# MiloszKrajewski/K4os.Compression.LZ4

Hardware: NVIDIA H100
Metric: GB/s uncompressed (encode+decode) on batched 64KiB blocks @1/2/4/8 GPU vs CPU ref (higher is better)
Workload: dtype u8

## Files before the change

k4os/compression/lz4_b200/csrc/encode_generic.cuh:

```cuda
#pragma once
#include "common.cuh"

namespace k4 {

constexpr int ENC_TABLE_BYTES = 16384;
constexpr int ENC_FLAG_X32 = 0x100;
#ifndef K4_ENC_TAGS
#define K4_ENC_TAGS 0
#endif
constexpr int ENC_TAG_BYTES = K4_ENC_TAGS ? 8192 : 0;
constexpr int ENC_SLOT_BYTES = ENC_TABLE_BYTES + ENC_TAG_BYTES;
#ifndef K4_ENC_GTAG
#define K4_ENC_GTAG 2
#endif
constexpr int ENC_GTAG = K4_ENC_GTAG;
constexpr int ENC_GSLOT_BYTES = ENC_GTAG == 2 ? 2 * ENC_TABLE_BYTES : (ENC_GTAG ? ENC_TABLE_BYTES + ENC_TABLE_BYTES / 2 : ENC_TABLE_BYTES);

struct EncCtx {
    const uint8_t* src;
    uint32_t n;
    bool by16;
    bool use5;
    uint16_t* t16;
    uint32_t* t32;
    __device__ __forceinline__ uint32_t hash_at(uint32_t p) const {
        if (by16) return hash4(ldg_u32u(src + p), 13);
        return use5 ? hash5(ldg_u64u(src + p), 12) : hash4(ldg_u32u(src + p), 12);
    }
    __device__ __forceinline__ uint32_t tget(uint32_t h) const { return by16 ? (uint32_t)t16[h] : t32[h]; }
    __device__ __forceinline__ void tput(uint32_t h, uint32_t v) const {
        if (by16) t16[h] = (uint16_t)v; else t32[h] = v;
    }
};

__device__ __forceinline__ uint32_t run_header_size(uint32_t run) {
    return run >= 15 ? 2 + (run - 15) / 255 : 1;
}
__device__ __forceinline__ void write_run_header(uint8_t* dst, uint32_t op, uint32_t run) {
    if (run >= 15) {
        uint32_t rest = run - 15;
        dst[op++] = 0xF0;
        for (; rest >= 255; rest -= 255) dst[op++] = 255;
        dst[op++] = (uint8_t)rest;
    } else {
        dst[op] = (uint8_t)(run << 4);
    }
}

__device__ int encode_block_warp(const uint8_t* __restrict__ src, int n_, uint8_t* __restrict__ dst,
                                 int cap, int hardCap, void* tableSmem, bool enforce32) {
    const int lane = lane_id();
    if ((uint32_t)n_ > (uint32_t)MAX_INPUT_SIZE) return 0;
    EncCtx c;
    c.src = src; c.n = (uint32_t)n_;
    c.by16 = n_ < LIMIT_64K;
    c.use5 = !c.by16 && !enforce32;
    c.t16 = reinterpret_cast<uint16_t*>(tableSmem);
    c.t32 = reinterpret_cast<uint32_t*>(tableSmem);
    const bool limited = !(cap >= max_output_size(n_));
    const int64_t olimit = cap;
    const int64_t hard = hardCap;
    const uint32_t n = c.n;

    {
        uint4* t = reinterpret_cast<uint4*>(tableSmem);
        for (int i = lane; i < ENC_TABLE_BYTES / 16; i += 32) t[i] = make_uint4(0, 0, 0, 0);
        __syncwarp();
    }

    uint32_t ip = 0, anchor = 0, op = 0;

    if (n >= (uint32_t)MINLENGTH) {
        const uint32_t mfl1 = n - MFLIMIT + 1;
        const uint32_t mlim = n - LASTLITERALS;
        uint32_t fh = 0, m = 0, tokpos = 0;
        if (lane == 0) {
            c.tput(c.hash_at(0), 0);
            fh = c.hash_at(1);
        }
        ip = 1;
        for (;;) {
            uint32_t status = 0;
            if (lane == 0) {
                uint32_t fwd = ip, step = 1, cnt = 1u << SKIP_TRIGGER;
                for (;;) {
                    const uint32_t hh = fh, cur = fwd;
                    m = c.tget(hh);
                    ip = fwd;
                    fwd += step;
                    step = cnt++ >> SKIP_TRIGGER;
                    if (fwd > mfl1) { status = 0; break; }
                    fh = c.hash_at(fwd);
                    c.tput(hh, cur);
                    if (!c.by16 && m + MAX_DISTANCE < cur) continue;
                    if (ldg_u32u(src + m) == ldg_u32u(src + ip)) { status = 1; break; }
                }
                if (status) {
                    while (ip > anchor && m > 0 && __ldg(src + ip - 1) == __ldg(src + m - 1)) { ip--; m--; }
                }
            }
            status = __shfl_sync(FULL, status, 0);
            if (!status) break;
            ip = __shfl_sync(FULL, ip, 0);
            m = __shfl_sync(FULL, m, 0);

            {
                const uint32_t lit = ip - anchor;
                if (limited && (int64_t)op + 1 + lit + 8 + lit / 255 > olimit) return 0;
                const uint32_t hdr = run_header_size(lit);
                if ((int64_t)op + hdr + lit > hard) return 0;
                tokpos = op;
                if (lane == 0) write_run_header(dst, op, lit);
                op += hdr;
                for (uint32_t i = lane; i < lit; i += 32) dst[op + i] = __ldg(src + anchor + i);
                op += lit;
            }

            for (;;) {
                if ((int64_t)op + 2 > hard) return 0;
                if (lane == 0) { dst[op] = (uint8_t)(ip - m); dst[op + 1] = (uint8_t)((ip - m) >> 8); }
                op += 2;
                uint32_t mc = 0;
                {
                    uint32_t a = ip + MINMATCH, b = m + MINMATCH;
                    for (;;) {
                        const bool in = a + lane < mlim;
                        const bool eq = in && (__ldg(src + a + lane) == __ldg(src + b + lane));
                        const unsigned miss = __ballot_sync(FULL, !eq);
                        if (miss) { mc += __ffs(miss) - 1; break; }
                        mc += 32; a += 32; b += 32;
                    }
                }
                ip += mc + MINMATCH;
                if (limited && (int64_t)op + 6 + (mc + 240) / 255 > olimit) return 0;
                if (mc >= 15) {
                    const uint32_t rest = mc - 15;
                    const uint32_t nff = rest / 255;
                    if ((int64_t)op + nff + 1 > hard) return 0;
                    for (uint32_t i = lane; i < nff; i += 32) dst[op + i] = 0xFF;
                    if (lane == 0) {
                        dst[tokpos] = (uint8_t)(dst[tokpos] + 15);
                        dst[op + nff] = (uint8_t)(rest % 255);
                    }
                    op += nff + 1;
                } else if (lane == 0) {
                    dst[tokpos] = (uint8_t)(dst[tokpos] + mc);
                }
                __syncwarp();
                anchor = ip;
                if (ip >= mfl1) goto last_literals;

                uint32_t hit = 0;
                if (lane == 0) {
                    c.tput(c.hash_at(ip - 2), ip - 2);
                    const uint32_t hh = c.hash_at(ip);
                    m = c.tget(hh);
                    c.tput(hh, ip);
                    if ((c.by16 || m + MAX_DISTANCE >= ip) && ldg_u32u(src + m) == ldg_u32u(src + ip))
                        hit = 1;
                    else
                        fh = c.hash_at(ip + 1);
                }
                hit = __shfl_sync(FULL, hit, 0);
                if (!hit) { ip++; break; }
                m = __shfl_sync(FULL, m, 0);
                if ((int64_t)op + 1 > hard) return 0;
                tokpos = op;
                if (lane == 0) dst[op] = 0;
                op++;
                __syncwarp();
            }
        }
    }

last_literals:
    {
        const uint32_t run = n - anchor;
        if (limited && (int64_t)op + run + 1 + (run + 255 - 15) / 255 > olimit) return 0;
        const uint32_t hdr = run_header_size(run);
        if ((int64_t)op + hdr + run > hard) return 0;
        if (lane == 0) write_run_header(dst, op, run);
        op += hdr;
        for (uint32_t i = lane; i < run; i += 32) dst[op + i] = __ldg(src + anchor + i);
        op += run;
    }
    return (int)op;
}

__device__ __forceinline__ int codec_encode_warp(const uint8_t* src, int n, uint8_t* dst, int cap,
                                                 int level, void* table, bool enforce32) {
    if (n <= 0) return 0;
    if (level >= 3) return -2;
    int r = encode_block_warp(src, n, dst, cap, 0x7fffffff, table, enforce32);
    return r <= 0 ? -1 : r;
}

constexpr int ENC_WARPS_PER_CTA = K4_ENC_TAGS ? 9 : 7;
#ifndef K4_ENC_SM_WARPS
#define K4_ENC_SM_WARPS 8
#endif
#ifndef K4_ENC_GM_WARPS
#define K4_ENC_GM_WARPS 22
#endif
constexpr int ENC_SM_WARPS = K4_ENC_SM_WARPS;
constexpr int ENC_GM_WARPS = K4_ENC_GM_WARPS;

}
```

k4os/compression/lz4_b200/csrc/encode_tile.cuh:

```cuda
#pragma once
#include "common.cuh"
#include "encode_generic.cuh"

namespace k4 {


__device__ __forceinline__ uint32_t lds_u32u(const uint8_t* p) {
    const uintptr_t a = reinterpret_cast<uintptr_t>(p);
    const uint32_t* w = reinterpret_cast<const uint32_t*>(a & ~uintptr_t(3));
    return __funnelshift_r(w[0], w[1], (uint32_t)(a & 3) * 8);
}

#ifndef K4_ENC_OVL
#define K4_ENC_OVL 1
#endif
#ifndef K4_ENC_PF
#define K4_ENC_PF 0
#endif
__device__ __forceinline__ void prefetch_l1(const void* p) { asm volatile("prefetch.global.L1 [%0];" :: "l"(p)); }

__device__ __forceinline__ uint32_t probe_advance(uint32_t q) {
    if (q <= 64u) return q;
    if (q == 0) return 0;
    const uint32_t c = 63u + q, k = c >> 6;
    return 1u + 32u * k * (k - 1u) + (c - 64u * k) * k;
}

template <bool STAGED, bool HARD = true, bool GTAB = false, int TAGMODE = (K4_ENC_TAGS ? 1 : 0)>
__device__ int encode_spec_warp(const uint8_t* __restrict__ src, const uint8_t* sin, const uint32_t n,
                                uint8_t* __restrict__ dst, const int cap, const int hardCap, uint16_t* table) {
    const int lane = lane_id();
    const int64_t hard = hardCap;
#define RD32(p) (STAGED ? lds_u32u(sin + (p)) : ldg_u32u(src + (p)))
#ifndef K4_ENC_GTAB_L1
#define K4_ENC_GTAB_L1 0
#endif
#define TGET(h) ((GTAB && !K4_ENC_GTAB_L1) ? (uint32_t)__ldcg(table + (h)) : (uint32_t)table[(h)])
    constexpr bool TAGS = TAGMODE != 0;
    constexpr uint32_t TAG_SHIFT = TAGMODE == 2 ? 3u : 11u, TAG_MASK = TAGMODE == 2 ? 0xFFFFu : 0xFFu;
    uint8_t* const tags = reinterpret_cast<uint8_t*>(table) + ENC_TABLE_BYTES;
    uint32_t* const table32 = reinterpret_cast<uint32_t*>(table);
    auto tagGet = [&](uint32_t h) -> uint32_t {
        return (GTAB && !K4_ENC_GTAB_L1) ? (uint32_t)__ldcg(tags + h) : (uint32_t)tags[h];
    };
    auto slotPut = [&](uint32_t h, uint32_t pos, uint32_t tg) {
        if (TAGMODE == 2) {
            if (GTAB) __stcg(table32 + h, pos | (tg << 16)); else table32[h] = pos | (tg << 16);
        } else {
            if (GTAB && !K4_ENC_GTAB_L1) __stcg(table + h, (uint16_t)pos); else table[h] = (uint16_t)pos;
            if (TAGS) { if (GTAB && !K4_ENC_GTAB_L1) __stcg(tags + h, (uint8_t)tg); else tags[h] = (uint8_t)tg; }
        }
    };
#define RD8(p) (STAGED ? (uint32_t)sin[(p)] : (uint32_t)__ldg(src + (p)))
    {
        const uint32_t t0 = (TAGS && n >= 4) ? (((RD32(0) * 2654435761u) >> TAG_SHIFT) & TAG_MASK) : 0u;
        const uint32_t fillT = TAGMODE == 2 ? (t0 << 16) : 0u;
        uint4* t = reinterpret_cast<uint4*>(table);
        constexpr int TBYTES = TAGMODE == 2 ? 2 * ENC_TABLE_BYTES : ENC_TABLE_BYTES;
        for (int i = lane; i < TBYTES / 16; i += 32) {
            if (GTAB) __stcg(t + i, make_uint4(fillT, fillT, fillT, fillT)); else t[i] = make_uint4(fillT, fillT, fillT, fillT);
        }
        if (TAGMODE == 1 || TAGMODE == 3) {
            const uint32_t b4 = t0 * 0x01010101u;
            uint4* g = reinterpret_cast<uint4*>(tags);
            for (int i = lane; i < (ENC_TABLE_BYTES / 2) / 16; i += 32) {
                if (GTAB) __stcg(g + i, make_uint4(b4, b4, b4, b4)); else g[i] = make_uint4(b4, b4, b4, b4);
            }
        }
        __syncwarp();
    }
    const bool limited = !(cap >= max_output_size((int)n));
    const int64_t olimit = cap;
    uint32_t ip = 0, anchor = 0, op = 0;

    if (n >= (uint32_t)MINLENGTH) {
        const uint32_t mfl1 = n - MFLIMIT + 1, mlim = n - LASTLITERALS;
        if (lane == 0) { const uint32_t p0 = RD32(0) * 2654435761u; slotPut(p0 >> 19, 0u, (p0 >> TAG_SHIFT) & TAG_MASK); }
        __syncwarp();
        ip = 1;
        bool post = false;
        uint32_t q0 = 0;
        uint32_t base = 1;
        for (;;) {
            uint32_t h2 = 0xFFFFFFFFu, tag2 = 0;
            if (post) { const uint32_t p2 = RD32(ip - 2) * 2654435761u; h2 = p2 >> 19; tag2 = (p2 >> TAG_SHIFT) & TAG_MASK; }
            const bool isPost = post && lane == 0;
            const uint32_t q = q0 + (uint32_t)lane - (post ? 1u : 0u);
            const uint32_t pos = isPost ? ip : base + probe_advance(q);
            const bool valid = isPost || (base + probe_advance(q + 1) <= mfl1);
            const uint32_t v = valid ? RD32(pos) : 0u;
            const uint32_t prod = v * 2654435761u;
            const uint32_t h = valid ? prod >> 19 : (0x10000u + (uint32_t)lane);
            const uint32_t tg = (prod >> TAG_SHIFT) & TAG_MASK;
            uint32_t cand = 0u, ctag = tg;
            bool lazyPos = false;
            if (TAGMODE == 2) {
                const uint32_t e32 = valid ? ((GTAB && !K4_ENC_GTAB_L1) ? __ldcg(table32 + h) : table32[h]) : 0xFFFF0000u;
                cand = e32 & 0xFFFFu; ctag = e32 >> 16;
                if (!valid) ctag = 0x10000u;
            } else if (TAGMODE == 3) {
                ctag = valid ? tagGet(h) : 0x100u;
                lazyPos = true;
            } else {
                cand = valid ? TGET(h) : 0u;
                if (TAGMODE == 1) ctag = valid ? tagGet(h) : 0x100u;
            }
            if (h == h2) { cand = ip - 2; ctag = TAGS ? tag2 : tg; lazyPos = false; }
            const unsigned peers = __match_any_sync(FULL, h);
            const unsigned earlier = peers & ((1u << lane) - 1u);
            const int fromLane = earlier ? 31 - __clz(earlier) : lane;
            const uint32_t fwdPos = __shfl_sync(FULL, pos, fromLane);
            const uint32_t fwdTag = __shfl_sync(FULL, tg, fromLane);
            if (earlier) { cand = fwdPos; ctag = TAGS ? fwdTag : tg; lazyPos = false; }
            bool hit = false;
            if (valid && ctag == tg) {
                if (TAGMODE == 3 && lazyPos) cand = TGET(h);
                hit = RD32(cand) == v;
                if (TAGS && !STAGED && (K4_ENC_PF & 1)) {
                    prefetch_l1(src + (cand + 32u < n ? cand + 32u : n - 1u));
                    if (cand >= 8u) prefetch_l1(src + cand - 8u);
                }
            }
            if (!STAGED && (K4_ENC_PF & 2) && lane == 0) prefetch_l1(src + (pos + 384u < n ? pos + 384u : n - 1u));
            const unsigned hits = __ballot_sync(FULL, hit);
            const unsigned ends = __ballot_sync(FULL, !valid);
            const int f = hits ? __ffs(hits) - 1 : 32;
            const int e = ends ? __ffs(ends) - 1 : 32;
            if (e < f) break;
            {
                const unsigned upto = (f >= 31) ? 0xffffffffu : ((2u << f) - 1u);
                const unsigned later = peers & ~((2u << lane) - 1u) & upto;
                const bool doStore = valid && ((1u << lane) & upto) && !(lane < 31 ? later : 0u);
                if (post) {
                    const unsigned same2 = __ballot_sync(FULL, valid && h == h2) & upto;
                    if (lane == 0 && !same2) {
                        slotPut(h2, ip - 2, tag2);
                    }
                }
                if (doStore) slotPut(h, pos, tg);
                __syncwarp();
            }
            if (f == 32) {
                if (post) { post = false; base = ip + 1; q0 = 31; }
                else q0 += 32;
                continue;
            }
            const bool zeroLit = post && f == 0;
            uint32_t m = __shfl_sync(FULL, cand, f);
            ip = __shfl_sync(FULL, pos, f);
            const uint32_t a0h = ip + MINMATCH, b0h = m + MINMATCH;
            uint32_t x1 = 0u;
            if (K4_ENC_OVL) {
                const uint32_t a = a0h + 4u * lane;
                if (lane < 8 && (int)mlim - (int)a > 0) x1 = RD32(a) ^ RD32(b0h + 4u * lane);
            }
            uint32_t caught = 0;
            if (!zeroLit) {
                for (int width = 8;; width = 32) {
                    const bool part = lane < width;
                    const bool ok = !part || ((ip > anchor + lane) && (m > (uint32_t)lane) &&
                                              (RD8(ip - 1 - lane) == RD8(m - 1 - lane)));
                    const unsigned bad = __ballot_sync(FULL, !ok);
                    const int c = bad ? __ffs(bad) - 1 : width;
                    ip -= c; m -= c; caught += (uint32_t)c;
                    if (bad) break;
                }
            }
            const uint32_t lit = ip - anchor;
            if (!zeroLit && limited && (int64_t)op + 1 + lit + 8 + lit / 255 > olimit) return 0;
            uint32_t mc = caught;
            {
                uint32_t a0 = a0h, b0 = b0h;
                for (int width = 8;; width = 32) {
                    const uint32_t a = a0 + 4u * lane, bb = b0 + 4u * lane;
                    const bool part = lane < width;
                    const int room = (int)mlim - (int)a;
                    const uint32_t x = (K4_ENC_OVL && width == 8) ? x1 : ((part && room > 0) ? (RD32(a) ^ RD32(bb)) : 0u);
                    int eq = x ? ((__ffs(x) - 1) >> 3) : 4;
                    if (eq > room) eq = room < 0 ? 0 : room;
                    if (!part) eq = 4;
                    const unsigned stop = __ballot_sync(FULL, eq < 4);
                    if (stop) {
                        const int s = __ffs(stop) - 1;
                        mc += 4u * s + (uint32_t)__shfl_sync(FULL, eq, s);
                        break;
                    }
                    mc += 4u * width; a0 += 4u * width; b0 += 4u * width;
                }
            }
            const uint32_t hdr = run_header_size(lit);
            const uint32_t afterOff = op + hdr + lit + 2;
            if (limited && (int64_t)afterOff + 6 + (mc + 240) / 255 > olimit) return 0;
            if (HARD && (int64_t)afterOff + (mc >= 15 ? (mc - 15) / 255 + 1 : 0) > hard) return 0;
            {
                const uint32_t mlTok = mc >= 15 ? 15u : mc;
                if (lane == 0) {
                    if (lit >= 15) {
                        uint32_t o = op, rest = lit - 15;
                        dst[o++] = (uint8_t)(0xF0 | mlTok);
                        for (; rest >= 255; rest -= 255) dst[o++] = 255;
                        dst[o] = (uint8_t)rest;
                    } else dst[op] = (uint8_t)((lit << 4) | mlTok);
                    dst[afterOff - 2] = (uint8_t)(ip - m);
                    dst[afterOff - 1] = (uint8_t)((ip - m) >> 8);
                }
                for (uint32_t i = lane; i < lit; i += 32) dst[op + hdr + i] = RD8(anchor + i);
                op = afterOff;
                if (mc >= 15) {
                    const uint32_t rest = mc - 15, nff = rest / 255;
                    for (uint32_t i = lane; i < nff; i += 32) dst[op + i] = 0xFF;
                    if (lane == 0) dst[op + nff] = (uint8_t)(rest % 255);
                    op += nff + 1;
                }
            }
            ip += mc + MINMATCH;
            anchor = ip;
            if (ip >= mfl1) break;
            post = true; q0 = 0; base = ip + 1;
        }
    }
    {
        const uint32_t run = n - anchor;
        if (limited && (int64_t)op + run + 1 + (run + 255 - 15) / 255 > olimit) return 0;
        const uint32_t hdr = run_header_size(run);
        if (HARD && (int64_t)op + hdr + run > hard) return 0;
        if (lane == 0) write_run_header(dst, op, run);
        op += hdr;
        for (uint32_t i = lane; i < run; i += 32) dst[op + i] = RD8(anchor + i);
        op += run;
        return (int)op;
    }
#undef RD32
#undef TGET
#undef RD8
}

__device__ unsigned long long g_encode_stats[4];

template <bool GTAB>
__device__ __forceinline__ void encode_persistent_warp(
        const uint8_t* __restrict__ srcBase, const int64_t* __restrict__ srcOff,
        const int32_t* __restrict__ srcLen, uint8_t* __restrict__ dstBase,
        const int64_t* __restrict__ dstOff, const int32_t* __restrict__ dstCap,
        int32_t* __restrict__ outLen, const int nBlocks, int level,
        uint32_t* __restrict__ nextBlock, uint16_t* const table, const int reserve) {
    const int lane = lane_id();
    const bool enforce32 = (level & ENC_FLAG_X32) != 0;
    level &= 0xFF;
    for (;;) {
        int b = 0;
        if (lane == 0) {
            if (GTAB && (int)*(volatile uint32_t*)nextBlock >= nBlocks - reserve) b = nBlocks;
            else b = (int)atomicAdd(nextBlock, 1u);
        }
        b = __shfl_sync(FULL, b, 0);
        if (b >= nBlocks) return;
        const int n_ = srcLen[b];
        const uint8_t* __restrict__ src = srcBase + srcOff[b];
        uint8_t* __restrict__ dst = dstBase + dstOff[b];
        const int cap = dstCap[b];
        if (n_ <= 0) { if (lane == 0) outLen[b] = 0; continue; }
        if (level >= 3) { if (lane == 0) outLen[b] = -2; continue; }
        int r;
        if (n_ >= LIMIT_64K) r = encode_block_warp(src, n_, dst, cap, 0x7fffffff, table, enforce32);
        else r = encode_spec_warp<false, false, GTAB, GTAB ? ENC_GTAG : (K4_ENC_TAGS ? 1 : 0)>(src, nullptr, (uint32_t)n_, dst, cap, 0x7fffffff, table);
        if (lane == 0) {
            outLen[b] = r <= 0 ? -1 : r;
            atomicAdd(&g_encode_stats[n_ >= LIMIT_64K ? 2 : (GTAB ? 1 : 0)], 1ull);
        }
        __syncwarp();
    }
}

__global__ void __launch_bounds__(32)
encode_spec_kernel(const uint8_t* __restrict__ srcBase, const int64_t* __restrict__ srcOff,
                   const int32_t* __restrict__ srcLen, uint8_t* __restrict__ dstBase,
                   const int64_t* __restrict__ dstOff, const int32_t* __restrict__ dstCap,
                   int32_t* __restrict__ outLen, int nBlocks, int level, uint32_t* __restrict__ nextBlock) {
    extern __shared__ __align__(128) uint8_t smem_encs[];
    encode_persistent_warp<false>(srcBase, srcOff, srcLen, dstBase, dstOff, dstCap, outLen, nBlocks, level,
                                  nextBlock, reinterpret_cast<uint16_t*>(smem_encs), 0);
}

__global__ void __launch_bounds__(32)
encode_spec_gtab_kernel(const uint8_t* __restrict__ srcBase, const int64_t* __restrict__ srcOff,
                        const int32_t* __restrict__ srcLen, uint8_t* __restrict__ dstBase,
                        const int64_t* __restrict__ dstOff, const int32_t* __restrict__ dstCap,
                        int32_t* __restrict__ outLen, int nBlocks, int level, uint32_t* __restrict__ nextBlock,
                        uint8_t* __restrict__ gtab, int reserve) {
    encode_persistent_warp<true>(srcBase, srcOff, srcLen, dstBase, dstOff, dstCap, outLen, nBlocks, level, nextBlock,
                                 reinterpret_cast<uint16_t*>(gtab + (size_t)blockIdx.x * ENC_GSLOT_BYTES), reserve);
}

}
```

Before: 48.87.

## Narrow first probe window after each match and speculatively verify tag-agreeing candidates

After each match, the first probe batch of the warp-parallel encoder now covers only 16 lanes (K4_ENC_WIN), so fewer table probes are wasted past the next likely hit. When tags are in use with overlap, verification of the full 4-byte match is speculative: lanes whose tags agree are visited in order, and the backward extension and first 32 match bytes are computed together with the verification, removing later shuffle and reload steps. The warp split between shared-memory and global-table encoders also moves from 8/22 to 10/20. The cost is serialized per-candidate loops when tags give false positives, and smaller probe batches that may need more iterations.

Result: faster. 51.72 (median of 6 runs) (+5.8%).

```diff
diff --git a/k4os/compression/lz4_b200/csrc/encode_generic.cuh b/k4os/compression/lz4_b200/csrc/encode_generic.cuh
--- a/k4os/compression/lz4_b200/csrc/encode_generic.cuh
+++ b/k4os/compression/lz4_b200/csrc/encode_generic.cuh
@@ -197,10 +197,10 @@
 
 constexpr int ENC_WARPS_PER_CTA = K4_ENC_TAGS ? 9 : 7;
 #ifndef K4_ENC_SM_WARPS
-#define K4_ENC_SM_WARPS 8
+#define K4_ENC_SM_WARPS 10
 #endif
 #ifndef K4_ENC_GM_WARPS
-#define K4_ENC_GM_WARPS 22
+#define K4_ENC_GM_WARPS 20
 #endif
 constexpr int ENC_SM_WARPS = K4_ENC_SM_WARPS;
 constexpr int ENC_GM_WARPS = K4_ENC_GM_WARPS;
diff --git a/k4os/compression/lz4_b200/csrc/encode_tile.cuh b/k4os/compression/lz4_b200/csrc/encode_tile.cuh
--- a/k4os/compression/lz4_b200/csrc/encode_tile.cuh
+++ b/k4os/compression/lz4_b200/csrc/encode_tile.cuh
@@ -17,6 +17,13 @@
 #ifndef K4_ENC_PF
 #define K4_ENC_PF 0
 #endif
+#ifndef K4_ENC_WIN
+#define K4_ENC_WIN 16
+#endif
+#ifndef K4_ENC_SPEC
+#define K4_ENC_SPEC 1
+#endif
+static_assert(K4_ENC_WIN >= 0 && K4_ENC_WIN <= 32, "K4_ENC_WIN: lanes of a run's first batch, 1..32 (0 = 32)");
 __device__ __forceinline__ void prefetch_l1(const void* p) { asm volatile("prefetch.global.L1 [%0];" :: "l"(p)); }
 
 __device__ __forceinline__ uint32_t probe_advance(uint32_t q) {
@@ -26,7 +33,7 @@
     return 1u + 32u * k * (k - 1u) + (c - 64u * k) * k;
 }
 
-template <bool STAGED, bool HARD = true, bool GTAB = false, int TAGMODE = (K4_ENC_TAGS ? 1 : 0)>
+template <bool STAGED, bool HARD = true, bool GTAB = false, int TAGMODE = (K4_ENC_TAGS ? 1 : 0), int WIN = 32>
 __device__ int encode_spec_warp(const uint8_t* __restrict__ src, const uint8_t* sin, const uint32_t n,
                                 uint8_t* __restrict__ dst, const int cap, const int hardCap, uint16_t* table) {
     const int lane = lane_id();
@@ -81,13 +88,17 @@
         bool post = false;
         uint32_t q0 = 0;
         uint32_t base = 1;
+        constexpr uint32_t WIN0 = (WIN <= 0 || WIN > 32) ? 32u : (uint32_t)WIN;
+        constexpr bool NARROW = WIN0 < 32u;
+        uint32_t width = WIN0;
         for (;;) {
             uint32_t h2 = 0xFFFFFFFFu, tag2 = 0;
             if (post) { const uint32_t p2 = RD32(ip - 2) * 2654435761u; h2 = p2 >> 19; tag2 = (p2 >> TAG_SHIFT) & TAG_MASK; }
             const bool isPost = post && lane == 0;
             const uint32_t q = q0 + (uint32_t)lane - (post ? 1u : 0u);
             const uint32_t pos = isPost ? ip : base + probe_advance(q);
-            const bool valid = isPost || (base + probe_advance(q + 1) <= mfl1);
+            const bool inWin = !NARROW || (uint32_t)lane < width;
+            const bool valid = inWin && (isPost || (base + probe_advance(q + 1) <= mfl1));
             const uint32_t v = valid ? RD32(pos) : 0u;
             const uint32_t prod = v * 2654435761u;
             const uint32_t h = valid ? prod >> 19 : (0x10000u + (uint32_t)lane);
@@ -112,8 +123,9 @@
             const uint32_t fwdPos = __shfl_sync(FULL, pos, fromLane);
             const uint32_t fwdTag = __shfl_sync(FULL, tg, fromLane);
             if (earlier) { cand = fwdPos; ctag = TAGS ? fwdTag : tg; lazyPos = false; }
+            constexpr bool SPEC = K4_ENC_SPEC && TAGMODE == 2 && K4_ENC_OVL;
             bool hit = false;
-            if (valid && ctag == tg) {
+            if (!SPEC && valid && ctag == tg) {
                 if (TAGMODE == 3 && lazyPos) cand = TGET(h);
                 hit = RD32(cand) == v;
                 if (TAGS && !STAGED && (K4_ENC_PF & 1)) {
@@ -122,10 +134,33 @@
                 }
             }
             if (!STAGED && (K4_ENC_PF & 2) && lane == 0) prefetch_l1(src + (pos + 384u < n ? pos + 384u : n - 1u));
-            const unsigned hits = __ballot_sync(FULL, hit);
-            const unsigned ends = __ballot_sync(FULL, !valid);
-            const int f = hits ? __ffs(hits) - 1 : 32;
+            const unsigned ends = __ballot_sync(FULL, inWin && !valid);
             const int e = ends ? __ffs(ends) - 1 : 32;
+            int f = 32;
+            uint32_t sm = 0u, sip = 0u, sx1 = 0u;
+            bool sok = true;
+            if (SPEC) {
+                for (unsigned agree = __ballot_sync(FULL, valid && ctag == tg); agree; agree &= agree - 1u) {
+                    const int c = __ffs(agree) - 1;
+                    if (e < c) break;
+                    sm = __shfl_sync(FULL, cand, c);
+                    sip = __shfl_sync(FULL, pos, c);
+                    const uint32_t vc = __shfl_sync(FULL, v, c);
+                    bool same = true;
+                    sx1 = 0u; sok = true;
+                    if (lane < 8) {
+                        const uint32_t a = sip + MINMATCH + 4u * lane;
+                        if ((int)mlim - (int)a > 0) sx1 = RD32(a) ^ RD32(sm + MINMATCH + 4u * lane);
+                        sok = (sip > anchor + lane) && (sm > (uint32_t)lane) && (RD8(sip - 1 - lane) == RD8(sm - 1 - lane));
+                    } else if (lane == 8) {
+                        same = RD32(sm) == vc;
+                    }
+                    if (__all_sync(FULL, same)) { f = c; break; }
+                }
+            } else {
+                const unsigned hits = __ballot_sync(FULL, hit);
+                f = hits ? __ffs(hits) - 1 : 32;
+            }
             if (e < f) break;
             {
                 const unsigned upto = (f >= 31) ? 0xffffffffu : ((2u << f) - 1u);
@@ -141,16 +176,18 @@
                 __syncwarp();
             }
             if (f == 32) {
-                if (post) { post = false; base = ip + 1; q0 = 31; }
-                else q0 += 32;
+                const uint32_t w = NARROW ? width : 32u;
+                if (post) { post = false; base = ip + 1; q0 = w - 1; }
+                else q0 += w;
+                width = 32;
                 continue;
             }
             const bool zeroLit = post && f == 0;
-            uint32_t m = __shfl_sync(FULL, cand, f);
-            ip = __shfl_sync(FULL, pos, f);
+            uint32_t m = SPEC ? sm : __shfl_sync(FULL, cand, f);
+            ip = SPEC ? sip : __shfl_sync(FULL, pos, f);
             const uint32_t a0h = ip + MINMATCH, b0h = m + MINMATCH;
-            uint32_t x1 = 0u;
-            if (K4_ENC_OVL) {
+            uint32_t x1 = sx1;
+            if (K4_ENC_OVL && !SPEC) {
                 const uint32_t a = a0h + 4u * lane;
                 if (lane < 8 && (int)mlim - (int)a > 0) x1 = RD32(a) ^ RD32(b0h + 4u * lane);
             }
@@ -158,8 +195,9 @@
             if (!zeroLit) {
                 for (int width = 8;; width = 32) {
                     const bool part = lane < width;
-                    const bool ok = !part || ((ip > anchor + lane) && (m > (uint32_t)lane) &&
-                                              (RD8(ip - 1 - lane) == RD8(m - 1 - lane)));
+                    const bool ok = (SPEC && width == 8) ? sok
+                                  : (!part || ((ip > anchor + lane) && (m > (uint32_t)lane) &&
+                                               (RD8(ip - 1 - lane) == RD8(m - 1 - lane))));
                     const unsigned bad = __ballot_sync(FULL, !ok);
                     const int c = bad ? __ffs(bad) - 1 : width;
                     ip -= c; m -= c; caught += (uint32_t)c;
@@ -216,7 +254,7 @@
             ip += mc + MINMATCH;
             anchor = ip;
             if (ip >= mfl1) break;
-            post = true; q0 = 0; base = ip + 1;
+            post = true; q0 = 0; base = ip + 1; width = WIN0;
         }
     }
     {
@@ -263,7 +301,7 @@
         if (level >= 3) { if (lane == 0) outLen[b] = -2; continue; }
         int r;
         if (n_ >= LIMIT_64K) r = encode_block_warp(src, n_, dst, cap, 0x7fffffff, table, enforce32);
-        else r = encode_spec_warp<false, false, GTAB, GTAB ? ENC_GTAG : (K4_ENC_TAGS ? 1 : 0)>(src, nullptr, (uint32_t)n_, dst, cap, 0x7fffffff, table);
+        else r = encode_spec_warp<false, false, GTAB, GTAB ? ENC_GTAG : (K4_ENC_TAGS ? 1 : 0), K4_ENC_WIN>(src, nullptr, (uint32_t)n_, dst, cap, 0x7fffffff, table);
         if (lane == 0) {
             outLen[b] = r <= 0 ? -1 : r;
             atomicAdd(&g_encode_stats[n_ >= LIMIT_64K ? 2 : (GTAB ? 1 : 0)], 1ull);
```
